# mpeg5/xeve

Measured on AMD Instinct MI355X. Metric: encoded frames/sec @ 2160p Baseline medium; SAD-kernel HBM GB/s vs peak, higher is better.
Workload: dtype s16 samples, s32/s64 accumulation, f64 cost comparisons (bit-exact)

## Files before the change

xeve_amd/csrc/tree.hip:

```cpp
#include <algorithm>
#include <atomic>
#include <cmath>
#include <cstdlib>
#include <cstring>
#include <vector>
#include "xh_common.h"
#include "cu_lane.h"

#define MAX_COST 1.7e+308
typedef xeve_hip_ctu_data CtuData;
typedef xeve_hip_sbac     SbacState;

struct Node {
    int    active, x0, y0, leaf, do_split, best_split, dist_cu, cu_mode, try_intra, next_split;
    double cost_best, cost_temp, unit_cost, cost_split;
};

#define XT_STREAMS 5
struct TreeK {
    int    nchains, log2_ctu, pic_w, pic_h, w_scu, h_scu, max_cu, min_cu, min_cuwh, idc, ws, hs, slice_qp, slice_num, s_mod_l, s_mod_c;
    long   mod_pic_l, mod_pic_c, map_pic;
    double lambda0;
    pel                        *mod[3];
    uint32_t                   *map_scu, *map_cu_mode;
    int8_t                     *map_ipm;
    const SbacState            *states;
    const xeve_hip_ctu_job     *jobs;
    CtuData                    *out;
    SbacState                  *out_next;
    double                     *out_cost;
    Node                       *node;
    SbacState                  *curr, *next, *before, *tdepth;
    CtuData                    *best, *temp;
    int                         inter, ecu_depth, s_org_l, vh;
    int16_t                   (*map_mv)[2][2];
    int8_t                    (*map_refi)[2];
    struct Ac {
        xeve_hip_intra_job          *ijobs;
        const xeve_hip_intra_result *ires;
        const int16_t               *icoef;
        const pel                   *irec;
        SbacState                   *sbest;
        xeve_hip_inter_job          *ejobs;
        xeve_hip_job                *sjobs;
        const xeve_hip_inter_result *eres;
        const int16_t               *ecoef;
        const pel                   *erec[3];
        const int32_t               *esatd;
        const SbacState             *enext;
    } ac[XT_STREAMS];
    unsigned char side_of[8];
    SbacState    *csplit;
    CtuData      *tsplit;
};

enum { OP_ENTER = 0, OP_LEAF = 1, OP_CHILD_DONE = 2, OP_EXIT = 3, OP_ROOT_DONE = 4, OP_MID = 5, OP_SPLIT_PREP = 6, OP_LEAF_SIDE = 7 };
#define MAX_OPS 12
struct OpList {
    int           n;
    unsigned char op[MAX_OPS], lvl[MAX_OPS];
    signed char   part[MAX_OPS];
};

__device__ static void bc_byte(SbacState &s, unsigned b)
{
    if(s.is_pending_byte) {
        if(s.pending_byte == 0) s.stacked_zero++;
        else s.bitcounter += 8 * s.stacked_zero + 8, s.stacked_zero = 0;
    }
    s.pending_byte = b & 0xFF, s.is_pending_byte = 1;
}
__device__ static void bc_shift(SbacState &s)
{
    s.code <<= 1;
    if(--s.code_bits) return;
    const unsigned out = s.code >> 17;
    s.code &= (1u << 17) - 1;
    if(out < 0xFF) {
        for(; s.stacked_ff; s.stacked_ff--) bc_byte(s, 0xFF);
        bc_byte(s, out);
    }
    else if(out > 0xFF) {
        s.pending_byte++;
        for(; s.stacked_ff; s.stacked_ff--) bc_byte(s, 0);
        bc_byte(s, out);
    }
    else s.stacked_ff++;
    s.code_bits = 8;
}
__device__ static unsigned split_flag_bits(const SbacState &from, SbacState &to, int split)
{
    SbacState s = from;
    s.code &= 0x7FFFF, s.code_bits = 11;
    s.pending_byte = s.is_pending_byte = s.stacked_ff = s.stacked_zero = s.bitcounter = s.bin_counter = 0;
    unsigned state = s.ctx[XEVE_HIP_CTX_SPLIT_CU] >> 1, mps = s.ctx[XEVE_HIP_CTX_SPLIT_CU] & 1;
    unsigned lps = (state * s.range) >> 9;
    if(lps < 437) lps = 437;
    s.bin_counter++;
    s.range -= lps;
    if((unsigned)(split != 0) != mps) {
        if(s.range >= lps) s.code += s.range, s.range = lps;
        state = state + ((512 - state + 16) >> 5);
        if(state > 256) mps = 1 - mps, state = 512 - state;
    }
    else state = state - ((state + 16) >> 5);
    s.ctx[XEVE_HIP_CTX_SPLIT_CU] = (uint16_t)((state << 1) + mps);
    while(s.range < 8192) s.range <<= 1, bc_shift(s);
    to = s;
    return s.bitcounter + 8 * (s.stacked_zero + s.stacked_ff) + 8 * (s.is_pending_byte ? 1 : 0) + 8 - s.code_bits + 3;
}

__device__ static unsigned split_flag_inplace(SbacState *st, int split)
{
    SbacState s;
    s.range = st->range, s.code = st->code & 0x7FFFF, s.code_bits = 11;
    s.pending_byte = s.is_pending_byte = s.stacked_ff = s.stacked_zero = s.bitcounter = s.bin_counter = 0;
    const unsigned m = st->ctx[XEVE_HIP_CTX_SPLIT_CU];
    unsigned state = m >> 1, mps = m & 1;
    unsigned lps = (state * s.range) >> 9;
    if(lps < 437) lps = 437;
    s.bin_counter++;
    s.range -= lps;
    if((unsigned)(split != 0) != mps) {
        if(s.range >= lps) s.code += s.range, s.range = lps;
        state = state + ((512 - state + 16) >> 5);
        if(state > 256) mps = 1 - mps, state = 512 - state;
    }
    else state = state - ((state + 16) >> 5);
    while(s.range < 8192) s.range <<= 1, bc_shift(s);
    st->range = s.range, st->code = s.code, st->code_bits = s.code_bits, st->stacked_ff = s.stacked_ff, st->stacked_zero = s.stacked_zero, st->pending_byte = s.pending_byte;
    st->is_pending_byte = s.is_pending_byte, st->bitcounter = s.bitcounter, st->bin_counter = s.bin_counter;
    st->ctx[XEVE_HIP_CTX_SPLIT_CU] = (uint16_t)((state << 1) + mps);
    return s.bitcounter + 8 * (s.stacked_zero + s.stacked_ff) + 8 * (s.is_pending_byte ? 1 : 0) + 8 - s.code_bits + 3;
}

static_assert(sizeof(SbacState) % 4 == 0, "coder states are moved word by word");
__device__ static void st_copy(SbacState *dst, const SbacState *src, SbacState *dst2 = nullptr)
{
    const unsigned *a = (const unsigned *)src;
    unsigned       *b = (unsigned *)dst, *b2 = (unsigned *)dst2;
    for(int i = threadIdx.x; i < (int)(sizeof(SbacState) / 4); i += blockDim.x) {
        const unsigned v = a[i];
        b[i] = v;
        if(b2) b2[i] = v;
    }
}
__device__ static void st_zero(SbacState *dst)
{
    unsigned *b = (unsigned *)dst;
    for(int i = threadIdx.x; i < (int)(sizeof(SbacState) / 4); i += blockDim.x) b[i] = 0;
}
__device__ static void cud_init(CtuData *d, int log2)
{
    const int n = 1 << (2 * (log2 - 2));
    for(int u = threadIdx.x; u < n; u += blockDim.x) {
        for(int k = 0; k < XEVE_HIP_CU_DEPTHS; k++) d->split_mode[k][u] = 0;
        d->ipm[0][u] = 0, d->ipm[1][u] = 0;
    }
}
__device__ static void cud_copy(CtuData *dst, const CtuData *src, int x, int y, int log2, int log2_cus, int cud, int idc, int ws, int hs)
{
    const int n = 1 << (log2 - 2), cus = 1 << (log2_cus - 2), cw = 1 << log2, cs = 1 << log2_cus;
    for(int u = threadIdx.x; u < n * n; u += blockDim.x) {
        const int j = u / n, i = u - j * n, di = ((y >> 2) + j) * cus + (x >> 2) + i, si = u;
        for(int k = cud; k < XEVE_HIP_CU_DEPTHS; k++) dst->split_mode[k][di] = src->split_mode[k][si];
        dst->pred_mode[di] = src->pred_mode[si], dst->ipm[0][di] = src->ipm[0][si], dst->ipm[1][di] = src->ipm[1][si], dst->depth[di] = src->depth[si];
        dst->map_scu[di] = src->map_scu[si], dst->map_cu_mode[di] = src->map_cu_mode[si];
        for(int c = 0; c < 3; c++) dst->nnz[c][di] = src->nnz[c][si];
        for(int k = 0; k < 4; k++) (&dst->mv[di][0][0])[k] = (&src->mv[si][0][0])[k], (&dst->mvd[di][0][0])[k] = (&src->mvd[si][0][0])[k];
        for(int k = 0; k < 2; k++) dst->refi[di][k] = src->refi[si][k], dst->mvp_idx[di][k] = src->mvp_idx[si][k];
    }
    for(int t = threadIdx.x; t < cw * cw; t += blockDim.x) {
        const int j = t >> log2, i = t & (cw - 1), d = (y + j) * cs + x + i;
        dst->coef[0][d] = src->coef[0][t], dst->reco[0][d] = src->reco[0][t];
    }
    if(idc) {
        const int wc = cw >> ws, hc = cw >> hs, sc = cs >> ws;
        for(int t = threadIdx.x; t < wc * hc; t += blockDim.x) {
            const int j = t / wc, i = t - j * wc, d = ((y >> hs) + j) * sc + (x >> ws) + i;
            dst->coef[1][d] = src->coef[1][t], dst->reco[1][d] = src->reco[1][t];
            dst->coef[2][d] = src->coef[2][t], dst->reco[2][d] = src->reco[2][t];
        }
    }
}
__device__ static void clear_map(const TreeK &K, int pic, int x, int y, int cu)
{
    const int w = (x + cu > K.pic_w ? K.pic_w - x : cu) >> 2, h = (y + cu > K.pic_h ? K.pic_h - y : cu) >> 2;
    uint32_t *ms = K.map_scu + (long)pic * K.map_pic, *mc = K.map_cu_mode + (long)pic * K.map_pic;
    for(int t = threadIdx.x; t < w * h; t += blockDim.x) {
        const int j = t / w, i = t - j * w, g = ((y >> 2) + j) * K.w_scu + (x >> 2) + i;
        ms[g] = 0, mc[g] = 0;
    }
}
__device__ static void update_map(const TreeK &K, int pic, const CtuData *d, int x, int y, int cu)
{
    const int w = (x + cu > K.pic_w ? K.pic_w - x : cu) >> 2, h = (y + cu > K.pic_h ? K.pic_h - y : cu) >> 2, n = cu >> 2;
    uint32_t *ms = K.map_scu + (long)pic * K.map_pic, *mc = K.map_cu_mode + (long)pic * K.map_pic;
    int8_t   *mi = K.map_ipm + (long)pic * K.map_pic;
    for(int t = threadIdx.x; t < w * h; t += blockDim.x) {
        const int j = t / w, i = t - j * w, g = ((y >> 2) + j) * K.w_scu + (x >> 2) + i, u = j * n + i;
        ms[g] = d->map_scu[u], mc[g] = d->map_cu_mode[u], mi[g] = d->ipm[0][u];
        if(K.inter) {
            const long gm = (long)pic * K.map_pic + g;
            for(int k = 0; k < 4; k++) (&K.map_mv[gm][0][0])[k] = (&d->mv[u][0][0])[k];
            K.map_refi[gm][0] = d->refi[u][0], K.map_refi[gm][1] = d->refi[u][1];
        }
    }
}
__device__ static void rec_to_pic(const TreeK &K, int pic, const CtuData *d, int x, int y, int cu)
{
    const int w = x + cu > K.pic_w ? K.pic_w - x : cu, h = y + cu > K.pic_h ? K.pic_h - y : cu;
    pel *m = K.mod[0] + (long)pic * K.mod_pic_l;
    for(int t = threadIdx.x; t < w * h; t += blockDim.x) {
        const int j = t / w, i = t - j * w;
        m[(long)(y + j) * K.s_mod_l + x + i] = d->reco[0][j * cu + i];
    }
    if(K.idc) {
        const int wc = w >> K.ws, hc = h >> K.hs, sc = cu >> K.ws;
        pel *mu = K.mod[1] + (long)pic * K.mod_pic_c, *mv = K.mod[2] + (long)pic * K.mod_pic_c;
        for(int t = threadIdx.x; t < wc * hc; t += blockDim.x) {
            const int  j = t / wc, i = t - j * wc;
            const long g = (long)((y >> K.hs) + j) * K.s_mod_c + (x >> K.ws) + i;
            mu[g] = d->reco[1][j * sc + i], mv[g] = d->reco[2][j * sc + i];
        }
    }
}

#define AT(arr, L) ((arr) + (long)(L) * K.nchains + c)

__device__ static void op_enter(const TreeK &K, int c, int L, int part, int *sh)
{
    const xeve_hip_ctu_job J = K.jobs[c];
    Node *nd = AT(K.node, L);
    const int log2 = L + 2, cu = 1 << log2;
    if(threadIdx.x == 0) {
        int active, x0, y0;
        if(part < 0) active = 1, x0 = J.x, y0 = J.y;
        else {
            const Node *p = AT(K.node, L + 1);
            x0 = p->x0 + (part & 1) * cu, y0 = p->y0 + (part >> 1) * cu;
            active = p->active && p->do_split && x0 < K.pic_w && y0 < K.pic_h;
        }
        const int boundary = active && !(x0 + cu <= K.pic_w && y0 + cu <= K.pic_h), leaf = active && !boundary && cu <= K.max_cu;
        nd->active = active, nd->x0 = x0, nd->y0 = y0, nd->leaf = leaf;
        const int jx = leaf ? x0 : max(0, min(J.x, K.pic_w - cu)), jy = leaf ? y0 : max(0, min(J.y, K.pic_h - cu));
        xeve_hip_intra_job ij;
        memset(&ij, 0, sizeof(ij));
        ij.x = jx, ij.y = jy, ij.inter_satd = 0xFFFFFFFFu, ij.sbac = c, ij.pic = J.pic;
        const TreeK::Ac &A = K.ac[K.side_of[L]];
        *AT(A.ijobs, L) = ij;
        if(K.inter) {
            xeve_hip_inter_job ej;
            memset(&ej, 0, sizeof(ej));
            ej.x = jx, ej.y = jy + J.pic * K.vh, ej.sbac = c;
            *AT(A.ejobs, L) = ej;
            *AT(A.sjobs, L) = xh_make_job((long)jy + (long)J.pic * K.vh, K.s_org_l, jx, c * cu * cu);
            nd->try_intra = 0, nd->cu_mode = 0, nd->unit_cost = MAX_COST;
        }
        sh[0] = active, sh[1] = leaf, sh[2] = boundary, sh[3] = x0, sh[4] = y0;
    }
    __syncthreads();
    const int active = sh[0], leaf = sh[1], boundary = sh[2], x0 = sh[3], y0 = sh[4];
    if(active) {
        const SbacState *src = part < 0 ? K.states + J.sbac : part == 0 ? AT(K.csplit, L + 1) : AT(K.next, L);
        st_copy(AT(K.curr, L), src, AT(K.before, L));
        st_zero(AT(K.tdepth, L));
    }
    __syncthreads();
    if(threadIdx.x == 0 && active) {
        nd->cost_best = MAX_COST, nd->best_split = 0, nd->do_split = 0, nd->dist_cu = 0;
        double cost_temp = 0.0;
        if(!boundary) {
            if(leaf) {
                if(cu > K.min_cuwh) cost_temp += (double)(int)split_flag_inplace(AT(K.curr, L), 0) * K.lambda0;
            }
            else cost_temp = MAX_COST;
        }
        nd->cost_temp = cost_temp;
    }
    if(active && !boundary) cud_init(AT(K.best, L), log2);
    if(leaf) clear_map(K, J.pic, x0, y0, cu);
}

__device__ static void unit_to_temp(const TreeK &K, CtuData *t, int log2, int cud, int n, int cu_mode, const int8_t *ipm, const int32_t *nnz, const xeve_hip_inter_result *R,
                                    const int16_t *cy, const int16_t *cu_, const int16_t *cv, const pel *ry, const pel *ru, const pel *rv, int n0, int n1)
{
    const uint32_t scu = ((uint32_t)K.slice_num & 0x7F) | ((uint32_t)K.slice_qp << 16) | (1u << 31) | (cu_mode == 0 ? 1u << 15 : 0) | (cu_mode == 2 ? 1u << 23 : 0);
    const uint32_t cum = ((uint32_t)log2 << 24) | ((uint32_t)log2 << 28);
    for(int u = threadIdx.x; u < n; u += blockDim.x) {
        t->pred_mode[u] = (uint8_t)cu_mode, t->depth[u] = (int8_t)cud;
        if(cu_mode == 0) t->ipm[0][u] = ipm[0], t->ipm[1][u] = K.idc ? ipm[1] : 0;
        t->nnz[0][u] = nnz[0], t->nnz[1][u] = K.idc ? nnz[1] : 0, t->nnz[2][u] = K.idc ? nnz[2] : 0;
        t->map_scu[u] = scu, t->map_cu_mode[u] = cum;
        for(int k = 0; k < 4; k++) (&t->mv[u][0][0])[k] = R ? (&R->mv[0][0])[k] : 0, (&t->mvd[u][0][0])[k] = R ? (&R->mvd[0][0])[k] : 0;
        for(int k = 0; k < 2; k++) t->refi[u][k] = R ? R->refi[k] : -1, t->mvp_idx[u][k] = R ? R->mvp_idx[k] : 0;
    }
    for(int i = threadIdx.x; i < n0; i += blockDim.x) t->coef[0][i] = cy[i], t->reco[0][i] = ry[i];
    if(K.idc)
        for(int i = threadIdx.x; i < n1; i += blockDim.x) t->coef[1][i] = cu_[i], t->reco[1][i] = ru[i], t->coef[2][i] = cv[i], t->reco[2][i] = rv[i];
}

__device__ static void op_mid(const TreeK &K, int c, int L)
{
    Node *nd = AT(K.node, L);
    if(!nd->leaf) return;
    const int log2 = L + 2, cu = 1 << log2, cud = 2 * (K.log2_ctu - log2), n = 1 << (2 * L), n0 = cu * cu, n1 = K.idc ? n0 >> (K.ws + K.hs) : 0;
    const TreeK::Ac &A = K.ac[K.side_of[L]];
    const xeve_hip_inter_result R = A.eres[c];
    unit_to_temp(K, AT(K.best, L), log2, cud, n, R.cu_mode, nullptr, R.nnz, &A.eres[c], A.ecoef + (long)c * n0, A.ecoef + (long)K.nchains * n0 + (long)c * n1,
                 A.ecoef + (long)K.nchains * (n0 + n1) + (long)c * n1, A.erec[0] + (long)c * n0, A.erec[1] + (long)c * n1, A.erec[2] + (long)c * n1, n0, n1);
    if(threadIdx.x == 0) {
        nd->unit_cost = R.cost, nd->cu_mode = R.cu_mode;
        nd->try_intra = R.nnz[0] != 0 || R.nnz[1] != 0 || R.nnz[2] != 0;
        if(nd->try_intra) AT(A.ijobs, L)->inter_satd = (uint32_t)A.esatd[c];
    }
}

__device__ static void leaf_decide(const TreeK &K, int c, int L, int *sh, bool to_pic)
{
    const xeve_hip_ctu_job J = K.jobs[c];
    Node *nd = AT(K.node, L);
    const int log2 = L + 2, cu = 1 << log2, cud = 2 * (K.log2_ctu - log2), n = 1 << (2 * L), n0 = cu * cu, n1 = K.idc ? n0 >> (K.ws + K.hs) : 0;
    CtuData *b = AT(K.best, L);
    const TreeK::Ac &A = K.ac[K.side_of[L]];
    const xeve_hip_intra_result R = A.ires[c];
    const int intra_wins = !K.inter || (nd->try_intra && R.cost < nd->unit_cost);
    if(intra_wins)
        unit_to_temp(K, b, log2, cud, n, 0, R.ipm, R.nnz, nullptr, A.icoef + (long)c * n0, A.icoef + (long)K.nchains * n0 + (long)c * n1,
                     A.icoef + (long)K.nchains * (n0 + n1) + (long)c * n1, A.irec + (long)c * n0, A.irec + (long)K.nchains * n0 + (long)c * n1,
                     A.irec + (long)K.nchains * (n0 + n1) + (long)c * n1, n0, n1);
    __syncthreads();
    if(threadIdx.x == 0) {
        if(intra_wins) nd->unit_cost = R.cost, nd->cu_mode = 0, nd->dist_cu = R.dist_cu;
        else nd->dist_cu = 0x7FFFFFFF;
        const double cost_temp = nd->cost_temp + nd->unit_cost;
        sh[0] = nd->cost_best > cost_temp;
        if(sh[0]) nd->cost_best = cost_temp, nd->best_split = 0;
        nd->cost_temp = nd->cost_best;
    }
    __syncthreads();
    const int better = sh[0];
    if(better) {
        st_copy(AT(K.tdepth, L), intra_wins ? A.sbest + c : A.enext + c);
        if(to_pic) rec_to_pic(K, J.pic, b, nd->x0, nd->y0, cu);
    }
    __syncthreads();
}
__device__ static int leaf_next_split(const TreeK &K, const Node *nd, int L)
{
    const int log2 = L + 2, cud = 2 * (K.log2_ctu - log2);
    int next_split = 1;
    if(nd->active && nd->cost_best != MAX_COST && K.inter && cud >= K.ecu_depth && nd->cu_mode == 2 ) next_split = 0;
    if(nd->active && nd->cost_best != MAX_COST && !K.inter) {
        const int th = 1 << (2 * log2 + 7);
        if(nd->dist_cu < th) {
            const int bits_inc = (2 * log2 >= 6 ? 2 : 0) + 8;
            if(nd->dist_cu < K.lambda0 * bits_inc) next_split = 0;
        }
    }
    return next_split;
}

__device__ static void op_leaf(const TreeK &K, int c, int L, int *sh)
{
    const xeve_hip_ctu_job J = K.jobs[c];
    Node *nd = AT(K.node, L);
    const int log2 = L + 2, cu = 1 << log2;
    const int active = nd->active, x0 = nd->x0, y0 = nd->y0;
    CtuData *t = AT(K.temp, L);
    if(nd->leaf) leaf_decide(K, c, L, sh, true);
    if(threadIdx.x == 0) {
        const int do_split = active && cu > 4 && leaf_next_split(K, nd, L) && cu > K.min_cu && cu > K.min_cuwh;
        nd->do_split = do_split;
        if(do_split) {
            SbacState run;
            nd->cost_temp = (double)(int)split_flag_bits(*AT(K.before, L), run, 1) * K.lambda0;
            *AT(K.curr, L) = run, *AT(K.csplit, L) = run;
        }
        sh[0] = do_split;
    }
    __syncthreads();
    const int do_split = sh[0];
    __syncthreads();
    if(do_split) {
        cud_init(t, log2);
        clear_map(K, J.pic, x0, y0, cu);
    }
}

__device__ static void op_split_prep(const TreeK &K, int c, int L, int *sh)
{
    const xeve_hip_ctu_job J = K.jobs[c];
    Node *nd = AT(K.node, L);
    const int log2 = L + 2, cu = 1 << log2;
    if(threadIdx.x == 0) {
        const int do_split = nd->active && cu > 4 && cu > K.min_cu && cu > K.min_cuwh;
        nd->do_split = do_split, nd->next_split = 1;
        if(do_split) {
            SbacState run;
            nd->cost_split = (double)(int)split_flag_bits(*AT(K.before, L), run, 1) * K.lambda0;
            *AT(K.csplit, L) = run;
        }
        sh[0] = do_split;
    }
    __syncthreads();
    const int do_split = sh[0];
    __syncthreads();
    if(do_split) {
        cud_init(AT(K.tsplit, L), log2);
        clear_map(K, J.pic, nd->x0, nd->y0, cu);
    }
}
__device__ static void op_leaf_side(const TreeK &K, int c, int L, int *sh)
{
    Node *nd = AT(K.node, L);
    if(nd->leaf) leaf_decide(K, c, L, sh, false);
    if(threadIdx.x == 0) nd->next_split = leaf_next_split(K, nd, L);
}

__device__ static void op_child_done(const TreeK &K, int c, int L, int part)
{
    const xeve_hip_ctu_job J = K.jobs[c];
    Node       *p  = AT(K.node, L);
    const Node *ch = AT(K.node, L - 1);
    if(!ch->active) return;
    const int log2 = L + 2, cud = 2 * (K.log2_ctu - log2), half = 1 << (log2 - 1);
    const int side = K.side_of[L];
    if(threadIdx.x == 0) (side ? p->cost_split : p->cost_temp) += ch->cost_best;
    cud_copy(side ? AT(K.tsplit, L) : AT(K.temp, L), AT(K.best, L - 1), ch->x0 - p->x0, ch->y0 - p->y0, log2 - 1, log2, cud, K.idc, K.ws, K.hs);
    update_map(K, J.pic, AT(K.best, L - 1), ch->x0, ch->y0, half);
    (void)part;
}

__device__ static void op_exit(const TreeK &K, int c, int L, int *sh)
{
    const xeve_hip_ctu_job J = K.jobs[c];
    Node *nd = AT(K.node, L);
    if(!nd->active) return;
    const int log2 = L + 2, cu = 1 << log2, cud = 2 * (K.log2_ctu - log2);
    const int side = K.side_of[L];
    if(threadIdx.x == 0) {
        const double cost_split = side ? nd->cost_split : nd->cost_temp;
        sh[0] = nd->do_split && (!side || nd->next_split) && nd->cost_best - 0.0001 > cost_split;
        if(sh[0]) nd->cost_best = cost_split, nd->best_split = 5 ;
    }
    __syncthreads();
    const int split_wins = sh[0];
    if(split_wins) st_copy(AT(K.tdepth, L), AT(K.next, L - 1));
    st_copy(AT(K.next, L), AT(K.tdepth, L));
    __syncthreads();
    CtuData *b = AT(K.best, L);
    if(split_wins) {
        cud_copy(b, side ? AT(K.tsplit, L) : AT(K.temp, L), 0, 0, log2, log2, cud, K.idc, K.ws, K.hs);
        __syncthreads();
    }
    rec_to_pic(K, J.pic, b, nd->x0, nd->y0, cu);
    if(cu >= 8 && threadIdx.x == 0) b->split_mode[cud][((cu >> 1) >> 2) * (cu >> 2) + ((cu >> 1) >> 2)] = (int8_t)nd->best_split;
}

__device__ static void op_root_done(const TreeK &K, int c, int L)
{
    const xeve_hip_ctu_job J = K.jobs[c];
    const Node    *nd = AT(K.node, L);
    const CtuData *b  = AT(K.best, L);
    update_map(K, J.pic, b, nd->x0, nd->y0, 1 << (L + 2));
    const uint32_t *s = (const uint32_t *)b;
    uint32_t       *d = (uint32_t *)(K.out + c);
    for(int i = threadIdx.x; i < (int)(sizeof(CtuData) / 4); i += blockDim.x) d[i] = s[i];
    if(threadIdx.x == 0) K.out_next[c] = *AT(K.next, L), K.out_cost[c] = nd->cost_best;
}

__global__ void __launch_bounds__(256) k_tree_ops(TreeK K, OpList ops)
{
    __shared__ int sh[8];
    const int c = blockIdx.x;
    for(int i = 0; i < ops.n; i++) {
        const int L = ops.lvl[i], part = ops.part[i];
        switch(ops.op[i]) {
        case OP_ENTER: op_enter(K, c, L, part, sh); break;
        case OP_LEAF: op_leaf(K, c, L, sh); break;
        case OP_CHILD_DONE: op_child_done(K, c, L, part); break;
        case OP_EXIT: op_exit(K, c, L, sh); break;
        case OP_MID: op_mid(K, c, L); break;
        case OP_SPLIT_PREP: op_split_prep(K, c, L, sh); break;
        case OP_LEAF_SIDE: op_leaf_side(K, c, L, sh); break;
        default: op_root_done(K, c, L); break;
        }
        __syncthreads();
    }
}

template <int LOG2> __global__ void __launch_bounds__(64) k_intra_lane(TreeK K, xl::Params P, const pel *org_y, const pel *org_u, const pel *org_v, const uint8_t *map_tidx,
                                                                        long org_pic_l, long org_pic_c)
{
    const int c = blockIdx.x, L = LOG2 - 2;
    if(c >= K.nchains || threadIdx.x != 0) return;
    const Node *nd = AT(K.node, L);
    if(!nd->leaf || (K.inter && !nd->try_intra)) return;
    const TreeK::Ac &A = K.ac[K.side_of[L]];
    const xeve_hip_intra_job J = *AT(A.ijobs, L);
    const int  n0 = 1 << (2 * LOG2), n1 = K.idc ? n0 >> (K.ws + K.hs) : 0;
    const pel *org[3] = {org_y + J.pic * org_pic_l, org_u ? org_u + J.pic * org_pic_c : nullptr, org_v ? org_v + J.pic * org_pic_c : nullptr};
    const pel *mod[3] = {K.mod[0] + J.pic * K.mod_pic_l, K.mod[1] ? K.mod[1] + J.pic * K.mod_pic_c : nullptr, K.mod[2] ? K.mod[2] + J.pic * K.mod_pic_c : nullptr};
    int16_t *coef = const_cast<int16_t *>(A.icoef);
    pel     *rec = const_cast<pel *>(A.irec);
    const long oy = (long)c * n0, ou = (long)K.nchains * n0 + (long)c * n1, ov = (long)K.nchains * (n0 + n1) + (long)c * n1;
    xeve_hip_intra_result R;
    xl::intra_cu<LOG2>(P, org, mod, K.map_scu + J.pic * K.map_pic, K.map_ipm + J.pic * K.map_pic, map_tidx + J.pic * K.map_pic, *AT(K.curr, L), J, R, coef + oy, coef + ou, coef + ov,
                       rec + oy, rec + ou, rec + ov, A.sbest[c]);
    const_cast<xeve_hip_intra_result *>(A.ires)[c] = R;
}

extern "C" int xeve_hip_satd_jobs(const pel *p1, int s1, const pel *p2, int s2, const xeve_hip_job *jobs, int njobs, const int32_t *cand_off, int ncand, int w, int h,
                                  int bit_depth, int32_t *out, void *stream);
static size_t al(size_t v) { return (v + 255) & ~(size_t)255; }
struct TreeLayout {
    size_t node, curr, next, before, tdepth, csplit, best, temp, tsplit, zero32, total, zero_from, zero_bytes;
    struct Ac {
        size_t sbest, ijobs, ires, icoef, irec, iws, iws_bytes, est;
        size_t ejobs, sjobs, eres, ecoef, erec[3], epred, esatd, enext, ews, ews_bytes;
    } ac[XT_STREAMS];
    unsigned char side_of[8];
};
static bool tree_params_ok(const xeve_hip_tree_params *p)
{
    if(!(p && p->log2_ctu >= 3 && p->log2_ctu <= 6 && p->pic_w > 0 && p->pic_h > 0 && (p->pic_w & 3) == 0 && (p->pic_h & 3) == 0 && xh_pow2(p->max_cu) &&
         xh_pow2(p->min_cu) && p->min_cu >= 4 && p->max_cu >= p->min_cu && p->min_cuwh >= 4 && xh_pow2(p->min_cuwh) && p->ip.w_scu == (p->pic_w + 3) >> 2 &&
         p->ip.h_scu == (p->pic_h + 3) >> 2 && (p->rdo_dbk == 0 || p->rdo_dbk == 1)))
        return false;
    const xeve_hip_intra_params &ip = p->ip;
    if(!(ip.tool_iqt == 0 && ip.bit_depth >= 8 && ip.bit_depth <= 14 && (ip.chroma_format_idc == 0 || ip.chroma_format_idc == 1 || ip.chroma_format_idc == 3) &&
         ip.slice_type >= 0 && ip.slice_type <= 2 && p->slice_qp >= 0 && p->slice_qp <= 127))
        return false;
    for(int k = 0; k < (ip.chroma_format_idc ? 3 : 1); k++)
        if(ip.qp[k] < 0 || ip.qp[k] > 51 + 6 * (ip.bit_depth - 8)) return false;
    return true;
}
static bool tree_inter_ok(const xeve_hip_tree_params *p, const xeve_hip_tree_inter *I)
{
    return I && (p->ip.slice_type == 0 || p->ip.slice_type == 1) && p->min_cu >= 4 && I->refp && I->map_mv && I->map_refi && I->col_mv0 && I->coef_l && I->coef_c &&
           (p->ip.slice_type == 1 || I->col_mv1) && I->ipar.rdo.slice_type == p->ip.slice_type && I->ipar.rdo.pic_w == p->pic_w && I->ipar.rdo.pic_h == p->pic_h &&
           I->ipar.rdo.chroma_format_idc == p->ip.chroma_format_idc && I->ipar.rdo.bit_depth == p->ip.bit_depth &&
           I->ipar.max_cand >= 1 && I->ipar.max_cand <= 4 && I->ipar.rdo.tool_iqt == 0 && I->ipar.rdo.num_refp[0] >= 1 && I->ipar.rdo.num_refp[0] <= XEVE_HIP_MAX_REFP &&
           (p->ip.slice_type == 1 || (I->ipar.rdo.num_refp[1] >= 1 && I->ipar.rdo.num_refp[1] <= I->ipar.rdo.num_refp[0])) && I->ipar.me.hpel_cnt >= 0 &&
           I->ipar.me.hpel_cnt <= 8 && I->ipar.me.qpel_cnt >= 0 && I->ipar.me.qpel_cnt <= 8;
}
static xeve_hip_intra_params level_params(const xeve_hip_tree_params *p, int log2)
{
    xeve_hip_intra_params ip = p->ip;
    ip.log2_cuw = ip.log2_cuh = log2;
    return ip;
}
static xeve_hip_inter_params level_inter_params(const xeve_hip_tree_inter *I, int log2)
{
    xeve_hip_inter_params ep = I->ipar;
    ep.rdo.log2_cuw = ep.rdo.log2_cuh = log2;
    return ep;
}
static xl::Params lane_params(const xeve_hip_tree_params *p, int log2, int s_org_l, int s_org_c, int s_mod_l, int s_mod_c)
{
    static const int q_scale[6] = {26214, 23302, 20560, 18396, 16384, 14764}, dq_scale[6] = {40, 45, 51, 57, 64, 71};
    xl::Params P;
    const xeve_hip_intra_params &ip = p->ip;
    const int idc = ip.chroma_format_idc, bd = ip.bit_depth, lc = log2 - (idc <= 2 ? 1 : 0);
    P.idc = idc, P.bd = bd, P.slice_type = ip.slice_type, P.cip = ip.constrained_intra_pred != 0, P.w_scu = ip.w_scu, P.h_scu = ip.h_scu;
    P.s_org_l = s_org_l, P.s_org_c = s_org_c, P.s_mod_l = s_mod_l, P.s_mod_c = s_mod_c;
    for(int c = 0; c < 3; c++) {
        const int q = ip.qp[c], log2_size = c ? lc : log2, tr_shift = 15 - bd - log2_size;
        P.qp[c] = q, P.q_scale[c] = q_scale[q % 6], P.dq_scale[c] = dq_scale[q % 6] << (q / 6), P.lambda[c] = ip.lambda[c];
        double e = (double)(1 << 15) * pow(2.0, -tr_shift);
        e = e / q_scale[q % 6] / (1 << (bd - 8));
// ... 623 lines not shown
```

Measured before the change: 18.74.

## Stage tree nodes, jobs and coder states in LDS and vectorize CTU copies

The tree-ops kernel now copies the node records, job, and intra/inter results for a chain into shared memory once at launch. It runs all ops on those shared copies and writes back only the node words that changed. Coder states are moved by the first wave, one word per lane, with a small forwarding cache so recently written states are read from LDS. cud_copy and unit_to_temp use wider 64/32-bit moves and fewer passes, which cuts global traffic and several block barriers. In exchange the kernel uses more LDS and more complex bookkeeping, with alignment assumptions enforced by static_asserts.

```diff
diff --git a/xeve_amd/csrc/tree.hip b/xeve_amd/csrc/tree.hip
--- a/xeve_amd/csrc/tree.hip
+++ b/xeve_amd/csrc/tree.hip
@@ -88,28 +88,6 @@
     else s.stacked_ff++;
     s.code_bits = 8;
 }
-__device__ static unsigned split_flag_bits(const SbacState &from, SbacState &to, int split)
-{
-    SbacState s = from;
-    s.code &= 0x7FFFF, s.code_bits = 11;
-    s.pending_byte = s.is_pending_byte = s.stacked_ff = s.stacked_zero = s.bitcounter = s.bin_counter = 0;
-    unsigned state = s.ctx[XEVE_HIP_CTX_SPLIT_CU] >> 1, mps = s.ctx[XEVE_HIP_CTX_SPLIT_CU] & 1;
-    unsigned lps = (state * s.range) >> 9;
-    if(lps < 437) lps = 437;
-    s.bin_counter++;
-    s.range -= lps;
-    if((unsigned)(split != 0) != mps) {
-        if(s.range >= lps) s.code += s.range, s.range = lps;
-        state = state + ((512 - state + 16) >> 5);
-        if(state > 256) mps = 1 - mps, state = 512 - state;
-    }
-    else state = state - ((state + 16) >> 5);
-    s.ctx[XEVE_HIP_CTX_SPLIT_CU] = (uint16_t)((state << 1) + mps);
-    while(s.range < 8192) s.range <<= 1, bc_shift(s);
-    to = s;
-    return s.bitcounter + 8 * (s.stacked_zero + s.stacked_ff) + 8 * (s.is_pending_byte ? 1 : 0) + 8 - s.code_bits + 3;
-}
-
 __device__ static unsigned split_flag_inplace(SbacState *st, int split)
 {
     SbacState s;
@@ -135,20 +113,34 @@
 }
 
 static_assert(sizeof(SbacState) % 4 == 0, "coder states are moved word by word");
-__device__ static void st_copy(SbacState *dst, const SbacState *src, SbacState *dst2 = nullptr)
-{
-    const unsigned *a = (const unsigned *)src;
-    unsigned       *b = (unsigned *)dst, *b2 = (unsigned *)dst2;
-    for(int i = threadIdx.x; i < (int)(sizeof(SbacState) / 4); i += blockDim.x) {
-        const unsigned v = a[i];
-        b[i] = v;
-        if(b2) b2[i] = v;
-    }
+#define ST_WORDS ((int)(sizeof(SbacState) / 4))
+static_assert(ST_WORDS <= 64, "a coder state is moved by the first wave of the block, one word per lane");
+static_assert(sizeof(Node) % 4 == 0 && sizeof(xeve_hip_ctu_job) % 4 == 0 && sizeof(xeve_hip_intra_result) % 4 == 0 && sizeof(xeve_hip_inter_result) % 4 == 0, "staged word by word");
+#define NODE_WORDS ((int)(sizeof(Node) / 4))
+#define ERES_WORDS ((int)(sizeof(xeve_hip_inter_result) / 4))
+static_assert(ERES_WORDS < 64 && sizeof(xeve_hip_intra_result) / 4 <= 64 && sizeof(xeve_hip_ctu_job) / 4 <= 64, "a record is staged by the first 64 threads of the block, one word each (blocks have 64 or 256)");
+
+struct Chip {
+    Node                  nd[5], nd0[5];
+    xeve_hip_ctu_job      job;
+    xeve_hip_intra_result ires;
+    xeve_hip_inter_result eres;
+    int                   esatd, ires_op, eres_op;
+    unsigned              st[ST_WORDS];
+    unsigned              fw[ST_WORDS];
+    unsigned              bf[ST_WORDS];
+    int                   sh[8];
+};
+struct Fwd {
+    const SbacState *fw = nullptr, *bf = nullptr;
+};
+__device__ static unsigned st_word(const Chip &S, const Fwd &F, const SbacState *src, int i)
+{
+    return src == F.fw ? S.fw[i] : src == F.bf ? S.bf[i] : ((const unsigned *)src)[i];
 }
 __device__ static void st_zero(SbacState *dst)
 {
-    unsigned *b = (unsigned *)dst;
-    for(int i = threadIdx.x; i < (int)(sizeof(SbacState) / 4); i += blockDim.x) b[i] = 0;
+    if((int)threadIdx.x < ST_WORDS) ((unsigned *)dst)[threadIdx.x] = 0;
 }
 __device__ static void cud_init(CtuData *d, int log2)
 {
@@ -158,28 +150,44 @@
         d->ipm[0][u] = 0, d->ipm[1][u] = 0;
     }
 }
-__device__ static void cud_copy(CtuData *dst, const CtuData *src, int x, int y, int log2, int log2_cus, int cud, int idc, int ws, int hs)
+static_assert(offsetof(CtuData, mv) % 8 == 0 && offsetof(CtuData, mvd) % 8 == 0 && offsetof(CtuData, coef) % 8 == 0 && offsetof(CtuData, reco) % 8 == 0 && sizeof(CtuData) % 8 == 0 &&
+              offsetof(CtuData, refi) % 2 == 0 && offsetof(CtuData, mvp_idx) % 2 == 0, "cud_copy moves vectors, rows and index pairs as one word each");
+__device__ static void cud_copy(CtuData *__restrict__ dst, const CtuData *__restrict__ src, int x, int y, int log2, int log2_cus, int cud, int idc, int ws, int hs)
 {
     const int n = 1 << (log2 - 2), cus = 1 << (log2_cus - 2), cw = 1 << log2, cs = 1 << log2_cus;
     for(int u = threadIdx.x; u < n * n; u += blockDim.x) {
-        const int j = u / n, i = u - j * n, di = ((y >> 2) + j) * cus + (x >> 2) + i, si = u;
-        for(int k = cud; k < XEVE_HIP_CU_DEPTHS; k++) dst->split_mode[k][di] = src->split_mode[k][si];
-        dst->pred_mode[di] = src->pred_mode[si], dst->ipm[0][di] = src->ipm[0][si], dst->ipm[1][di] = src->ipm[1][si], dst->depth[di] = src->depth[si];
-        dst->map_scu[di] = src->map_scu[si], dst->map_cu_mode[di] = src->map_cu_mode[si];
-        for(int c = 0; c < 3; c++) dst->nnz[c][di] = src->nnz[c][si];
-        for(int k = 0; k < 4; k++) (&dst->mv[di][0][0])[k] = (&src->mv[si][0][0])[k], (&dst->mvd[di][0][0])[k] = (&src->mvd[si][0][0])[k];
-        for(int k = 0; k < 2; k++) dst->refi[di][k] = src->refi[si][k], dst->mvp_idx[di][k] = src->mvp_idx[si][k];
-    }
-    for(int t = threadIdx.x; t < cw * cw; t += blockDim.x) {
-        const int j = t >> log2, i = t & (cw - 1), d = (y + j) * cs + x + i;
-        dst->coef[0][d] = src->coef[0][t], dst->reco[0][d] = src->reco[0][t];
+        const int j = u >> (log2 - 2), i = u - j * n, di = ((y >> 2) + j) * cus + (x >> 2) + i, si = u;
+        int8_t sm[XEVE_HIP_CU_DEPTHS];
+#pragma unroll
+        for(int k = 0; k < XEVE_HIP_CU_DEPTHS; k++) sm[k] = k >= cud ? src->split_mode[k][si] : 0;
+        const uint8_t  pm = src->pred_mode[si];
+        const int8_t   i0 = src->ipm[0][si], i1 = src->ipm[1][si], dp = src->depth[si];
+        const uint32_t ms = src->map_scu[si], mc = src->map_cu_mode[si];
+        const int32_t  z0 = src->nnz[0][si], z1 = src->nnz[1][si], z2 = src->nnz[2][si];
+        const uint64_t mv = *(const uint64_t *)&src->mv[si][0][0], md = *(const uint64_t *)&src->mvd[si][0][0];
+        const uint16_t rf = *(const uint16_t *)&src->refi[si][0], mp = *(const uint16_t *)&src->mvp_idx[si][0];
+#pragma unroll
+        for(int k = 0; k < XEVE_HIP_CU_DEPTHS; k++)
+            if(k >= cud) dst->split_mode[k][di] = sm[k];
+        dst->pred_mode[di] = pm, dst->ipm[0][di] = i0, dst->ipm[1][di] = i1, dst->depth[di] = dp;
+        dst->map_scu[di] = ms, dst->map_cu_mode[di] = mc;
+        dst->nnz[0][di] = z0, dst->nnz[1][di] = z1, dst->nnz[2][di] = z2;
+        *(uint64_t *)&dst->mv[di][0][0] = mv, *(uint64_t *)&dst->mvd[di][0][0] = md;
+        *(uint16_t *)&dst->refi[di][0] = rf, *(uint16_t *)&dst->mvp_idx[di][0] = mp;
+    }
+    for(int t = threadIdx.x; t < (cw * cw) >> 2; t += blockDim.x) {
+        const int j = t >> (log2 - 2), i = (t & ((cw >> 2) - 1)) << 2, d = (y + j) * cs + x + i, s = j * cw + i;
+        const uint64_t a = *(const uint64_t *)&src->coef[0][s], b = *(const uint64_t *)&src->reco[0][s];
+        *(uint64_t *)&dst->coef[0][d] = a, *(uint64_t *)&dst->reco[0][d] = b;
     }
     if(idc) {
-        const int wc = cw >> ws, hc = cw >> hs, sc = cs >> ws;
-        for(int t = threadIdx.x; t < wc * hc; t += blockDim.x) {
-            const int j = t / wc, i = t - j * wc, d = ((y >> hs) + j) * sc + (x >> ws) + i;
-            dst->coef[1][d] = src->coef[1][t], dst->reco[1][d] = src->reco[1][t];
-            dst->coef[2][d] = src->coef[2][t], dst->reco[2][d] = src->reco[2][t];
+        const int wc = cw >> ws, hc = cw >> hs, sc = cs >> ws, w2 = wc >> 1;
+        for(int t = threadIdx.x; t < w2 * hc; t += blockDim.x) {
+            const int j = t / w2, i = (t - j * w2) << 1, d = ((y >> hs) + j) * sc + (x >> ws) + i, s = j * wc + i;
+            const uint32_t a = *(const uint32_t *)&src->coef[1][s], b = *(const uint32_t *)&src->reco[1][s];
+            const uint32_t e = *(const uint32_t *)&src->coef[2][s], f = *(const uint32_t *)&src->reco[2][s];
+            *(uint32_t *)&dst->coef[1][d] = a, *(uint32_t *)&dst->reco[1][d] = b;
+            *(uint32_t *)&dst->coef[2][d] = e, *(uint32_t *)&dst->reco[2][d] = f;
         }
     }
 }
@@ -199,11 +207,19 @@
     int8_t   *mi = K.map_ipm + (long)pic * K.map_pic;
     for(int t = threadIdx.x; t < w * h; t += blockDim.x) {
         const int j = t / w, i = t - j * w, g = ((y >> 2) + j) * K.w_scu + (x >> 2) + i, u = j * n + i;
-        ms[g] = d->map_scu[u], mc[g] = d->map_cu_mode[u], mi[g] = d->ipm[0][u];
+        const uint32_t a = d->map_scu[u], b = d->map_cu_mode[u];
+        const int8_t   m = d->ipm[0][u];
+        int16_t v[4] = {0, 0, 0, 0};
+        int8_t  r0 = 0, r1 = 0;
+        if(K.inter) {
+            for(int k = 0; k < 4; k++) v[k] = (&d->mv[u][0][0])[k];
+            r0 = d->refi[u][0], r1 = d->refi[u][1];
+        }
+        ms[g] = a, mc[g] = b, mi[g] = m;
         if(K.inter) {
             const long gm = (long)pic * K.map_pic + g;
-            for(int k = 0; k < 4; k++) (&K.map_mv[gm][0][0])[k] = (&d->mv[u][0][0])[k];
-            K.map_refi[gm][0] = d->refi[u][0], K.map_refi[gm][1] = d->refi[u][1];
+            for(int k = 0; k < 4; k++) (&K.map_mv[gm][0][0])[k] = v[k];
+            K.map_refi[gm][0] = r0, K.map_refi[gm][1] = r1;
         }
     }
 }
@@ -221,23 +237,25 @@
         for(int t = threadIdx.x; t < wc * hc; t += blockDim.x) {
             const int  j = t / wc, i = t - j * wc;
             const long g = (long)((y >> K.hs) + j) * K.s_mod_c + (x >> K.ws) + i;
-            mu[g] = d->reco[1][j * sc + i], mv[g] = d->reco[2][j * sc + i];
+            const pel  a = d->reco[1][j * sc + i], b = d->reco[2][j * sc + i];
+            mu[g] = a, mv[g] = b;
         }
     }
 }
 
 #define AT(arr, L) ((arr) + (long)(L) * K.nchains + c)
 
-__device__ static void op_enter(const TreeK &K, int c, int L, int part, int *sh)
-{
-    const xeve_hip_ctu_job J = K.jobs[c];
-    Node *nd = AT(K.node, L);
+__device__ static void op_enter(const TreeK &K, Chip &S, Fwd &F, int c, int L, int part)
+{
+    const xeve_hip_ctu_job J = S.job;
+    Node *nd = &S.nd[L];
+    int  *sh = S.sh;
     const int log2 = L + 2, cu = 1 << log2;
     if(threadIdx.x == 0) {
         int active, x0, y0;
         if(part < 0) active = 1, x0 = J.x, y0 = J.y;
         else {
-            const Node *p = AT(K.node, L + 1);
+            const Node *p = &S.nd[L + 1];
             x0 = p->x0 + (part & 1) * cu, y0 = p->y0 + (part >> 1) * cu;
             active = p->active && p->do_split && x0 < K.pic_w && y0 < K.pic_h;
         }
@@ -257,33 +275,40 @@
             *AT(A.sjobs, L) = xh_make_job((long)jy + (long)J.pic * K.vh, K.s_org_l, jx, c * cu * cu);
             nd->try_intra = 0, nd->cu_mode = 0, nd->unit_cost = MAX_COST;
         }
+        if(active) {
+            nd->cost_best = MAX_COST, nd->best_split = 0, nd->do_split = 0, nd->dist_cu = 0;
+            nd->cost_temp = boundary || leaf ? 0.0 : MAX_COST;
+        }
         sh[0] = active, sh[1] = leaf, sh[2] = boundary, sh[3] = x0, sh[4] = y0;
     }
     __syncthreads();
     const int active = sh[0], leaf = sh[1], boundary = sh[2], x0 = sh[3], y0 = sh[4];
     if(active) {
         const SbacState *src = part < 0 ? K.states + J.sbac : part == 0 ? AT(K.csplit, L + 1) : AT(K.next, L);
-        st_copy(AT(K.curr, L), src, AT(K.before, L));
+        const bool flag = leaf && cu > K.min_cuwh;
+        if((int)threadIdx.x < ST_WORDS) {
+            const int      i = threadIdx.x;
+            const unsigned v = st_word(S, F, src, i);
+            ((unsigned *)AT(K.before, L))[i] = v, S.bf[i] = v;
+            if(flag) S.st[i] = v;
+            else ((unsigned *)AT(K.curr, L))[i] = v;
+        }
+        F.bf = AT(K.before, L);
         st_zero(AT(K.tdepth, L));
-    }
-    __syncthreads();
-    if(threadIdx.x == 0 && active) {
-        nd->cost_best = MAX_COST, nd->best_split = 0, nd->do_split = 0, nd->dist_cu = 0;
-        double cost_temp = 0.0;
-        if(!boundary) {
-            if(leaf) {
-                if(cu > K.min_cuwh) cost_temp += (double)(int)split_flag_inplace(AT(K.curr, L), 0) * K.lambda0;
-            }
-            else cost_temp = MAX_COST;
-        }
-        nd->cost_temp = cost_temp;
+        if(flag) {
+            __syncthreads();
+            if(threadIdx.x == 0) nd->cost_temp = (double)(int)split_flag_inplace((SbacState *)S.st, 0) * K.lambda0;
+            __syncthreads();
+            if((int)threadIdx.x < ST_WORDS) ((unsigned *)AT(K.curr, L))[threadIdx.x] = S.st[threadIdx.x];
+        }
     }
     if(active && !boundary) cud_init(AT(K.best, L), log2);
     if(leaf) clear_map(K, J.pic, x0, y0, cu);
 }
 
-__device__ static void unit_to_temp(const TreeK &K, CtuData *t, int log2, int cud, int n, int cu_mode, const int8_t *ipm, const int32_t *nnz, const xeve_hip_inter_result *R,
-                                    const int16_t *cy, const int16_t *cu_, const int16_t *cv, const pel *ry, const pel *ru, const pel *rv, int n0, int n1)
+__device__ static void unit_to_temp(const TreeK &K, CtuData *__restrict__ t, int log2, int cud, int n, int cu_mode, const int8_t *ipm, const int32_t *nnz, const xeve_hip_inter_result *R,
+                                    const int16_t *__restrict__ cy, const int16_t *__restrict__ cu_, const int16_t *__restrict__ cv, const pel *__restrict__ ry,
+                                    const pel *__restrict__ ru, const pel *__restrict__ rv, int n0, int n1)
 {
     const uint32_t scu = ((uint32_t)K.slice_num & 0x7F) | ((uint32_t)K.slice_qp << 16) | (1u << 31) | (cu_mode == 0 ? 1u << 15 : 0) | (cu_mode == 2 ? 1u << 23 : 0);
     const uint32_t cum = ((uint32_t)log2 << 24) | ((uint32_t)log2 << 28);
@@ -295,36 +320,47 @@
         for(int k = 0; k < 4; k++) (&t->mv[u][0][0])[k] = R ? (&R->mv[0][0])[k] : 0, (&t->mvd[u][0][0])[k] = R ? (&R->mvd[0][0])[k] : 0;
         for(int k = 0; k < 2; k++) t->refi[u][k] = R ? R->refi[k] : -1, t->mvp_idx[u][k] = R ? R->mvp_idx[k] : 0;
     }
-    for(int i = threadIdx.x; i < n0; i += blockDim.x) t->coef[0][i] = cy[i], t->reco[0][i] = ry[i];
-    if(K.idc)
-        for(int i = threadIdx.x; i < n1; i += blockDim.x) t->coef[1][i] = cu_[i], t->reco[1][i] = ru[i], t->coef[2][i] = cv[i], t->reco[2][i] = rv[i];
-}
-
-__device__ static void op_mid(const TreeK &K, int c, int L)
-{
-    Node *nd = AT(K.node, L);
+    for(int i = threadIdx.x; i < n0; i += blockDim.x) {
+        const int16_t a = cy[i];
+        const pel     b = ry[i];
+        int16_t e = 0, g = 0;
+        pel     f = 0, h = 0;
+        const bool ch = K.idc && i < n1;
+        if(ch) e = cu_[i], f = ru[i], g = cv[i], h = rv[i];
+        t->coef[0][i] = a, t->reco[0][i] = b;
+        if(ch) t->coef[1][i] = e, t->reco[1][i] = f, t->coef[2][i] = g, t->reco[2][i] = h;
+    }
+}
+
+__device__ static void op_mid(const TreeK &K, Chip &S, int c, int L, int at)
+{
+    Node *nd = &S.nd[L];
     if(!nd->leaf) return;
     const int log2 = L + 2, cu = 1 << log2, cud = 2 * (K.log2_ctu - log2), n = 1 << (2 * L), n0 = cu * cu, n1 = K.idc ? n0 >> (K.ws + K.hs) : 0;
     const TreeK::Ac &A = K.ac[K.side_of[L]];
-    const xeve_hip_inter_result R = A.eres[c];
-    unit_to_temp(K, AT(K.best, L), log2, cud, n, R.cu_mode, nullptr, R.nnz, &A.eres[c], A.ecoef + (long)c * n0, A.ecoef + (long)K.nchains * n0 + (long)c * n1,
+    const bool staged = S.eres_op == at;
+    const xeve_hip_inter_result R = staged ? S.eres : A.eres[c];
+    unit_to_temp(K, AT(K.best, L), log2, cud, n, R.cu_mode, nullptr, R.nnz, &R, A.ecoef + (long)c * n0, A.ecoef + (long)K.nchains * n0 + (long)c * n1,
                  A.ecoef + (long)K.nchains * (n0 + n1) + (long)c * n1, A.erec[0] + (long)c * n0, A.erec[1] + (long)c * n1, A.erec[2] + (long)c * n1, n0, n1);
     if(threadIdx.x == 0) {
         nd->unit_cost = R.cost, nd->cu_mode = R.cu_mode;
         nd->try_intra = R.nnz[0] != 0 || R.nnz[1] != 0 || R.nnz[2] != 0;
-        if(nd->try_intra) AT(A.ijobs, L)->inter_satd = (uint32_t)A.esatd[c];
-    }
-}
-
-__device__ static void leaf_decide(const TreeK &K, int c, int L, int *sh, bool to_pic)
-{
-    const xeve_hip_ctu_job J = K.jobs[c];
-    Node *nd = AT(K.node, L);
+        if(nd->try_intra) AT(A.ijobs, L)->inter_satd = (uint32_t)(staged ? S.esatd : A.esatd[c]);
+    }
+}
+
+__device__ static void leaf_decide(const TreeK &K, Chip &S, int c, int L, int at, bool to_pic)
+{
+    const xeve_hip_ctu_job J = S.job;
+    Node *nd = &S.nd[L];
+    int  *sh = S.sh;
     const int log2 = L + 2, cu = 1 << log2, cud = 2 * (K.log2_ctu - log2), n = 1 << (2 * L), n0 = cu * cu, n1 = K.idc ? n0 >> (K.ws + K.hs) : 0;
     CtuData *b = AT(K.best, L);
     const TreeK::Ac &A = K.ac[K.side_of[L]];
-    const xeve_hip_intra_result R = A.ires[c];
+    const xeve_hip_intra_result R = S.ires_op == at ? S.ires : A.ires[c];
     const int intra_wins = !K.inter || (nd->try_intra && R.cost < nd->unit_cost);
+    unsigned stw = 0;
+    if((int)threadIdx.x < ST_WORDS) stw = ((const unsigned *)(intra_wins ? A.sbest + c : A.enext + c))[threadIdx.x];
     if(intra_wins)
         unit_to_temp(K, b, log2, cud, n, 0, R.ipm, R.nnz, nullptr, A.icoef + (long)c * n0, A.icoef + (long)K.nchains * n0 + (long)c * n1,
                      A.icoef + (long)K.nchains * (n0 + n1) + (long)c * n1, A.irec + (long)c * n0, A.irec + (long)K.nchains * n0 + (long)c * n1,
@@ -341,7 +377,7 @@
     __syncthreads();
     const int better = sh[0];
     if(better) {
-        st_copy(AT(K.tdepth, L), intra_wins ? A.sbest + c : A.enext + c);
+        if((int)threadIdx.x < ST_WORDS) ((unsigned *)AT(K.tdepth, L))[threadIdx.x] = stw;
         if(to_pic) rec_to_pic(K, J.pic, b, nd->x0, nd->y0, cu);
     }
     __syncthreads();
@@ -361,81 +397,82 @@
     return next_split;
 }
 
-__device__ static void op_leaf(const TreeK &K, int c, int L, int *sh)
-{
-    const xeve_hip_ctu_job J = K.jobs[c];
-    Node *nd = AT(K.node, L);
+__device__ static void split_state(const TreeK &K, Chip &S, Fwd &F, int c, int L, bool to_curr, double *cost)
+{
+    if((int)threadIdx.x < ST_WORDS) S.st[threadIdx.x] = st_word(S, F, AT(K.before, L), threadIdx.x);
+    __syncthreads();
+    if(threadIdx.x == 0) *cost = (double)(int)split_flag_inplace((SbacState *)S.st, 1) * K.lambda0;
+    __syncthreads();
+    if((int)threadIdx.x < ST_WORDS) {
+        const unsigned v = S.st[threadIdx.x];
+        ((unsigned *)AT(K.csplit, L))[threadIdx.x] = v, S.fw[threadIdx.x] = v;
+        if(to_curr) ((unsigned *)AT(K.curr, L))[threadIdx.x] = v;
+    }
+    F.fw = AT(K.csplit, L);
+}
+
+__device__ static void op_leaf(const TreeK &K, Chip &S, Fwd &F, int c, int L, int at)
+{
+    const xeve_hip_ctu_job J = S.job;
+    Node *nd = &S.nd[L];
+    int  *sh = S.sh;
     const int log2 = L + 2, cu = 1 << log2;
-    const int active = nd->active, x0 = nd->x0, y0 = nd->y0;
     CtuData *t = AT(K.temp, L);
-    if(nd->leaf) leaf_decide(K, c, L, sh, true);
+    if(nd->leaf) leaf_decide(K, S, c, L, at, true);
     if(threadIdx.x == 0) {
-        const int do_split = active && cu > 4 && leaf_next_split(K, nd, L) && cu > K.min_cu && cu > K.min_cuwh;
+        const int do_split = nd->active && cu > 4 && leaf_next_split(K, nd, L) && cu > K.min_cu && cu > K.min_cuwh;
         nd->do_split = do_split;
-        if(do_split) {
-            SbacState run;
-            nd->cost_temp = (double)(int)split_flag_bits(*AT(K.before, L), run, 1) * K.lambda0;
-            *AT(K.curr, L) = run, *AT(K.csplit, L) = run;
-        }
         sh[0] = do_split;
     }
     __syncthreads();
-    const int do_split = sh[0];
-    __syncthreads();
+    const int do_split = sh[0], x0 = nd->x0, y0 = nd->y0;
     if(do_split) {
+        split_state(K, S, F, c, L, true, &nd->cost_temp);
         cud_init(t, log2);
         clear_map(K, J.pic, x0, y0, cu);
     }
 }
 
-__device__ static void op_split_prep(const TreeK &K, int c, int L, int *sh)
-{
-    const xeve_hip_ctu_job J = K.jobs[c];
-    Node *nd = AT(K.node, L);
+__device__ static void op_split_prep(const TreeK &K, Chip &S, Fwd &F, int c, int L)
+{
+    const xeve_hip_ctu_job J = S.job;
+    Node *nd = &S.nd[L];
     const int log2 = L + 2, cu = 1 << log2;
-    if(threadIdx.x == 0) {
-        const int do_split = nd->active && cu > 4 && cu > K.min_cu && cu > K.min_cuwh;
-        nd->do_split = do_split, nd->next_split = 1;
-        if(do_split) {
-            SbacState run;
-            nd->cost_split = (double)(int)split_flag_bits(*AT(K.before, L), run, 1) * K.lambda0;
-            *AT(K.csplit, L) = run;
-        }
-        sh[0] = do_split;
-    }
-    __syncthreads();
-    const int do_split = sh[0];
-    __syncthreads();
+    const int do_split = nd->active && cu > 4 && cu > K.min_cu && cu > K.min_cuwh;
+    if(threadIdx.x == 0) nd->do_split = do_split, nd->next_split = 1;
     if(do_split) {
+        split_state(K, S, F, c, L, false, &nd->cost_split);
         cud_init(AT(K.tsplit, L), log2);
         clear_map(K, J.pic, nd->x0, nd->y0, cu);
     }
 }
-__device__ static void op_leaf_side(const TreeK &K, int c, int L, int *sh)
-{
-    Node *nd = AT(K.node, L);
-    if(nd->leaf) leaf_decide(K, c, L, sh, false);
+__device__ static void op_leaf_side(const TreeK &K, Chip &S, int c, int L, int at)
+{
+    Node *nd = &S.nd[L];
+    if(nd->leaf) leaf_decide(K, S, c, L, at, false);
     if(threadIdx.x == 0) nd->next_split = leaf_next_split(K, nd, L);
 }
 
-__device__ static void op_child_done(const TreeK &K, int c, int L, int part)
-{
-    const xeve_hip_ctu_job J = K.jobs[c];
-    Node       *p  = AT(K.node, L);
-    const Node *ch = AT(K.node, L - 1);
+__device__ static void op_child_done(const TreeK &K, Chip &S, int c, int L, int part)
+{
+    const xeve_hip_ctu_job J = S.job;
+    Node       *p  = &S.nd[L];
+    const Node *ch = &S.nd[L - 1];
     if(!ch->active) return;
     const int log2 = L + 2, cud = 2 * (K.log2_ctu - log2), half = 1 << (log2 - 1);
     const int side = K.side_of[L];
+    const int cx = ch->x0, cy = ch->y0, px = p->x0, py = p->y0;
     if(threadIdx.x == 0) (side ? p->cost_split : p->cost_temp) += ch->cost_best;
-    cud_copy(side ? AT(K.tsplit, L) : AT(K.temp, L), AT(K.best, L - 1), ch->x0 - p->x0, ch->y0 - p->y0, log2 - 1, log2, cud, K.idc, K.ws, K.hs);
-    update_map(K, J.pic, AT(K.best, L - 1), ch->x0, ch->y0, half);
+    cud_copy(side ? AT(K.tsplit, L) : AT(K.temp, L), AT(K.best, L - 1), cx - px, cy - py, log2 - 1, log2, cud, K.idc, K.ws, K.hs);
+    update_map(K, J.pic, AT(K.best, L - 1), cx, cy, half);
     (void)part;
 }
 
-__device__ static void op_exit(const TreeK &K, int c, int L, int *sh)
-{
-    const xeve_hip_ctu_job J = K.jobs[c];
-    Node *nd = AT(K.node, L);
+__device__ static void op_exit(const TreeK &K, Chip &S, Fwd &F, int c, int L)
+{
+    const xeve_hip_ctu_job J = S.job;
+    Node *nd = &S.nd[L];
+    int  *sh = S.sh;
     if(!nd->active) return;
     const int log2 = L + 2, cu = 1 << log2, cud = 2 * (K.log2_ctu - log2);
     const int side = K.side_of[L];
@@ -445,48 +482,91 @@
         if(sh[0]) nd->cost_best = cost_split, nd->best_split = 5 ;
     }
     __syncthreads();
-    const int split_wins = sh[0];
-    if(split_wins) st_copy(AT(K.tdepth, L), AT(K.next, L - 1));
-    st_copy(AT(K.next, L), AT(K.tdepth, L));
+    const int split_wins = sh[0], x0 = nd->x0, y0 = nd->y0;
+    if((int)threadIdx.x < ST_WORDS) {
+        const int i = threadIdx.x;
+        unsigned  v;
+        if(split_wins) v = st_word(S, F, AT(K.next, L - 1), i), ((unsigned *)AT(K.tdepth, L))[i] = v;
+        else v = ((const unsigned *)AT(K.tdepth, L))[i];
+        ((unsigned *)AT(K.next, L))[i] = v, S.fw[i] = v;
+    }
+    F.fw = AT(K.next, L);
+    CtuData *b = AT(K.best, L);
+    const CtuData *w = b;
+    if(split_wins) {
+        w = side ? AT(K.tsplit, L) : AT(K.temp, L);
+        cud_copy(b, w, 0, 0, log2, log2, cud, K.idc, K.ws, K.hs);
+    }
+    rec_to_pic(K, J.pic, w, x0, y0, cu);
     __syncthreads();
-    CtuData *b = AT(K.best, L);
-    if(split_wins) {
-        cud_copy(b, side ? AT(K.tsplit, L) : AT(K.temp, L), 0, 0, log2, log2, cud, K.idc, K.ws, K.hs);
-        __syncthreads();
-    }
-    rec_to_pic(K, J.pic, b, nd->x0, nd->y0, cu);
     if(cu >= 8 && threadIdx.x == 0) b->split_mode[cud][((cu >> 1) >> 2) * (cu >> 2) + ((cu >> 1) >> 2)] = (int8_t)nd->best_split;
 }
 
-__device__ static void op_root_done(const TreeK &K, int c, int L)
-{
-    const xeve_hip_ctu_job J = K.jobs[c];
-    const Node    *nd = AT(K.node, L);
+__device__ static void op_root_done(const TreeK &K, Chip &S, const Fwd &F, int c, int L)
+{
+    const xeve_hip_ctu_job J = S.job;
+    const Node    *nd = &S.nd[L];
     const CtuData *b  = AT(K.best, L);
+    if((int)threadIdx.x < ST_WORDS) ((unsigned *)(K.out_next + c))[threadIdx.x] = st_word(S, F, AT(K.next, L), threadIdx.x);
     update_map(K, J.pic, b, nd->x0, nd->y0, 1 << (L + 2));
     const uint32_t *s = (const uint32_t *)b;
     uint32_t       *d = (uint32_t *)(K.out + c);
     for(int i = threadIdx.x; i < (int)(sizeof(CtuData) / 4); i += blockDim.x) d[i] = s[i];
-    if(threadIdx.x == 0) K.out_next[c] = *AT(K.next, L), K.out_cost[c] = nd->cost_best;
+    if(threadIdx.x == 0) K.out_cost[c] = nd->cost_best;
 }
 
 __global__ void __launch_bounds__(256) k_tree_ops(TreeK K, OpList ops)
 {
-    __shared__ int sh[8];
-    const int c = blockIdx.x;
+    __shared__ Chip S;
+    Fwd       F;
+    const int c = blockIdx.x, tid = threadIdx.x;
+    unsigned lv = 0;
+    int      ires_op = -1, eres_op = -1;
+    for(int i = 0; i < ops.n; i++) {
+        const int L = ops.lvl[i], o = ops.op[i];
+        lv |= 1u << L;
+        if(o == OP_ENTER && ops.part[i] >= 0) lv |= 2u << L;
+        if(o == OP_CHILD_DONE) lv |= 1u << (L - 1);
+        if((o == OP_LEAF || o == OP_LEAF_SIDE) && ires_op < 0) ires_op = i;
+        if(o == OP_MID && eres_op < 0) eres_op = i;
+    }
+    lv &= 31u;
+    for(int i = tid; i < 5 * NODE_WORDS; i += blockDim.x) {
+        const int l = i / NODE_WORDS;
+        if(lv >> l & 1) {
+            const unsigned v = ((const unsigned *)AT(K.node, l))[i - l * NODE_WORDS];
+            ((unsigned *)S.nd)[i] = v, ((unsigned *)S.nd0)[i] = v;
+        }
+    }
+    if(tid < (int)(sizeof(xeve_hip_ctu_job) / 4)) ((unsigned *)&S.job)[tid] = ((const unsigned *)(K.jobs + c))[tid];
+    if(ires_op >= 0 && tid < (int)(sizeof(xeve_hip_intra_result) / 4)) ((unsigned *)&S.ires)[tid] = ((const unsigned *)(K.ac[K.side_of[ops.lvl[ires_op]]].ires + c))[tid];
+    if(eres_op >= 0) {
+        const TreeK::Ac &A = K.ac[K.side_of[ops.lvl[eres_op]]];
+        if(tid < ERES_WORDS) ((unsigned *)&S.eres)[tid] = ((const unsigned *)(A.eres + c))[tid];
+        if(tid == ERES_WORDS) S.esatd = A.esatd[c];
+    }
+    if(tid == 0) S.ires_op = ires_op, S.eres_op = eres_op;
+    __syncthreads();
     for(int i = 0; i < ops.n; i++) {
         const int L = ops.lvl[i], part = ops.part[i];
         switch(ops.op[i]) {
-        case OP_ENTER: op_enter(K, c, L, part, sh); break;
-        case OP_LEAF: op_leaf(K, c, L, sh); break;
-        case OP_CHILD_DONE: op_child_done(K, c, L, part); break;
-        case OP_EXIT: op_exit(K, c, L, sh); break;
-        case OP_MID: op_mid(K, c, L); break;
-        case OP_SPLIT_PREP: op_split_prep(K, c, L, sh); break;
-        case OP_LEAF_SIDE: op_leaf_side(K, c, L, sh); break;
-        default: op_root_done(K, c, L); break;
+        case OP_ENTER: op_enter(K, S, F, c, L, part); break;
+        case OP_LEAF: op_leaf(K, S, F, c, L, i); break;
+        case OP_CHILD_DONE: op_child_done(K, S, c, L, part); break;
+        case OP_EXIT: op_exit(K, S, F, c, L); break;
+        case OP_MID: op_mid(K, S, c, L, i); break;
+        case OP_SPLIT_PREP: op_split_prep(K, S, F, c, L); break;
+        case OP_LEAF_SIDE: op_leaf_side(K, S, c, L, i); break;
+        default: op_root_done(K, S, F, c, L); break;
         }
         __syncthreads();
+    }
+    for(int i = tid; i < 5 * NODE_WORDS; i += blockDim.x) {
+        const int l = i / NODE_WORDS;
+        if(lv >> l & 1) {
+            const unsigned v = ((const unsigned *)S.nd)[i];
+            if(v != ((const unsigned *)S.nd0)[i]) ((unsigned *)AT(K.node, l))[i - l * NODE_WORDS] = v;
+        }
     }
 }
 
```

New measurement: 19.43 (median of 6 runs). 3.7% higher.
